# michel-aractingi/soloRL

Hardware: AMD Instinct MI355X
Metric: env-steps/s (whole node) Solo12 walk, 4096 envs/GPU (higher is better)
Workload: dtype f32

## Files before the change

### solorl_amd/csrc/dynamics.hpp

```cpp
#pragma once
#include <utility>

#include "../../include/solorl.h"
#include "../../include/solorl_model_data.h"
#include "spatial.hpp"

namespace solo {

constexpr int MAX_CONTACTS = 8;
constexpr int MAX_LIMITS = 4;
constexpr int LIM_SLOT_ROWS = 2;
constexpr int MAX_ROWS = LIM_SLOT_ROWS + 3 * MAX_CONTACTS;
SD int extra_limits(int nlt) { return nlt > LIM_SLOT_ROWS ? nlt - LIM_SLOT_ROWS : 0; }
SD int contact_cap(int nlt) { return MAX_CONTACTS - extra_limits(nlt); }
constexpr int ROW_CORE = 20;
constexpr int NPRIM = 24;
constexpr double LIMIT_WINDOW = 0.0;
constexpr double DISC_EPS2 = 1e-12;
constexpr double DISC_RIM = 0.1;

#if defined(SOLO_WAVE_TIMING) && !defined(SOLO_HOST_SHIM)
constexpr int SOLO_WT_WAVES = 65536, SOLO_WT_FIELDS = 32;
__device__ unsigned long long solo_wave_times[SOLO_WT_WAVES][SOLO_WT_FIELDS];
__shared__ unsigned long long solo_pt_acc[16];
#define SOLO_PT_DECL() long long pt_last_ = 0
#define SOLO_PT_BEGIN() do { __builtin_amdgcn_s_waitcnt(0); pt_last_ = clock64(); } while (0)
#define SOLO_PT(i) do { __builtin_amdgcn_s_waitcnt(0); if (threadIdx.x == 0) { const long long n_ = clock64(); solo_pt_acc[i] += (unsigned long long)(n_ - pt_last_); } pt_last_ = clock64(); } while (0)
#else
#define SOLO_PT_DECL() do {} while (0)
#define SOLO_PT_BEGIN() do {} while (0)
#define SOLO_PT(i) do {} while (0)
#endif

template <int N, typename F, int... I>
SD void static_for_impl(F&& f, std::integer_sequence<int, I...>) { (f(std::integral_constant<int, I>{}), ...); }
template <int N, typename F> SD void static_for(F&& f) { static_for_impl<N>(f, std::make_integer_sequence<int, N>{}); }

template <int ROBOT> struct Robot;
template <> struct Robot<0> {
  static constexpr int NJ = 2, NQ = 8, NL = 13;
  static constexpr bool SHOULDER = false;
  static constexpr const solorl_model_data& MD = SOLORL_MODEL_SOLO8;
};
template <> struct Robot<1> {
  static constexpr int NJ = 3, NQ = 12, NL = 17;
  static constexpr bool SHOULDER = true;
  static constexpr const solorl_model_data& MD = SOLORL_MODEL_SOLO12;
};

constexpr bool base_points_are_sign_patterns(const solorl_model_data& md) {
  const solorl_prim_data& a = md.prims[0]; const solorl_prim_data& b = md.prims[8];
  for (int p = 0; p < 12; p++) {
    const solorl_prim_data& q = md.prims[p];
    const bool plate = p >= 8;
    const double sx = ((plate ? (p - 8) >> 1 : p >> 2) & 1) ? -1.0 : 1.0, sy = ((plate ? (p - 8) : p >> 1) & 1) ? -1.0 : 1.0;
    const double cx = (plate ? b.center[0] : a.center[0]) * sx, cy = (plate ? b.center[1] : a.center[1]) * sy;
    const double cz = plate ? b.center[2] : ((p & 1) ? -a.center[2] : a.center[2]);
    if (q.link != 0 || q.axis != -1 || q.center[0] != cx || q.center[1] != cy || q.center[2] != cz || q.margin != a.margin || q.friction != a.friction) return false;
  }
  return true;
}

template <typename T> struct PhysParams {
  T dt, gravity, erp, slop, warm, damping, vmax, qlim, inv_dt;
  int iterations;
  T tm_hw, tm_mu;
  T resid_thr;
  T cerp;
  T cmargin;
  int mode;
  enum { M_PIPE = 1, M_URDF = 2, M_CONE = 4, M_TREADMILL = 8 };
  SD bool pgs_pipe() const { return mode & M_PIPE; }
  SD bool urdf_inertia() const { return mode & M_URDF; }
  SD bool cone() const { return mode & M_CONE; }
  SD bool tm_on() const { return mode & M_TREADMILL; }
  void set_mode(bool pipe, bool urdf, bool cone_, bool treadmill) {
    mode = (pipe ? M_PIPE : 0) | (urdf ? M_URDF : 0) | (cone_ ? M_CONE : 0) | (treadmill ? M_TREADMILL : 0);
  }
};
template <typename T> PhysParams<T> make_phys(const solorl_config& c) {
  PhysParams<T> p;
  p.dt = (T)c.sim_dt; p.gravity = (T)c.gravity; p.erp = (T)c.erp; p.slop = (T)c.linear_slop; p.warm = (T)c.warmstart;
  p.damping = (T)c.damping; p.vmax = (T)c.max_velocity; p.qlim = (T)c.joint_limit; p.inv_dt = (T)(1.0 / c.sim_dt);
  p.iterations = c.solver_iterations;
  p.tm_hw = (T)c.treadmill_half_width; p.tm_mu = (T)c.treadmill_friction;
  p.resid_thr = c.solver_residual_threshold > 0 ? (T)std::sqrt(c.solver_residual_threshold) : T(-1);
  p.cerp = (T)c.contact_erp; p.cmargin = (T)c.collision_margin;
  p.set_mode(true, c.use_urdf_inertia != 0, c.friction_model == SOLORL_FRICTION_CONE, c.use_treadmill != 0);
  return p;
}
SD int strip_feet_bits(int smask) {
  return (((smask >> 13) & 1) << 24) | (((smask >> 15) & 1) << 25) | (((smask >> 17) & 1) << 26) | (((smask >> 19) & 1) << 27);
}

template <typename T, int NQ> struct PhysState {
  V3<T> pos; T qx, qy, qz, qw; V3<T> v, w;
  T q[NQ], qd[NQ];
};

template <typename T> struct JointF { SV<T> S, U, c; T Dinv, u; };

#ifndef SOLO_HOST_SHIM
extern __shared__ __attribute__((aligned(16))) unsigned char solo_smem_sym[];
#if defined(SOLO_WAVE_TIMING)
constexpr unsigned SOLO_LDS_BASE = 128;
// ... 1812 lines not shown
    T nz = cw * z + ax * yq - ay * x + az * ww;
    T nq = cw * ww - ax * x - ay * yq - az * z;
    T inv = rsqrt_fast(nx * nx + ny * ny + nz * nz + nq * nq);
    C.ps.qx = nx * inv; C.ps.qy = ny * inv; C.ps.qz = nz * inv; C.ps.qw = nq * inv;
  }
}

template <typename T, int ROBOT, typename LDS> struct TeamCtx {
  using type = CtxLds<T, ROBOT, TeamRows<T, LDS>::off_ctx>;
  static constexpr size_t bytes = TeamRows<T, LDS>::off_ctx + 4 * sizeof(SubCtx<T, ROBOT>);
};

template <typename T, int ROBOT, typename LDS, typename CH>
SNI_SCALAR void duo_helper_rates(CH ch, const PhysParams<T> pp, const LDS lds, int t, bool valid) {
  if (valid) phase_legrates_team<T, ROBOT, LDS, CH>(ch, pp, lds, t);
  WG_SYNC();
}

template <typename T, int ROBOT>
SNI_SCALAR void duo_join_rows() {
  WG_SYNC();
}

template <typename T, int ROBOT, typename LDS, typename CH>
SNI_SCALAR void duo_integrate_joints(CH ch, const PhysParams<T> pp, const LDS lds, int t, bool valid) {
  using RB = Robot<ROBOT>;
  using TRW = TeamRows<T, LDS>;
  constexpr int NJ = RB::NJ, LN = LDS::LANES;
  if (!valid) return;
  SubCtx<T, ROBOT>& C = ch.get();
  const T dt = pp.dt;
  const int mask = C.mask;
  const int nlt = C.nlim_total;
  const T* hdr = lds.hdr();
  const SV<T> w{{hdr[2 * LN], hdr[3 * LN], hdr[4 * LN]}, {hdr[5 * LN], hdr[6 * LN], hdr[7 * LN]}};
  const int tj = t < RB::NQ ? t : 0;
  const int L = tj / NJ, k = tj - L * NJ;
  const T qds = C.qds[tj], yk = lds.y()[(L * 3 + k) * LN], qj = C.ps.q[tj];
  const SV<T> Gk = C.LR[L].G[k];
  const T* lam = TRW::lam(lds.lane);
  const int npos0 = TRW::NPOS0 + extra_limits(nlt);
  T lv[(NPRIM + 15) / 16];
#pragma unroll
  for (int i = 0; i < (NPRIM + 15) / 16; i++) {
    const int p = t + 16 * i;
    const int pp_ = p < NPRIM ? p : 0;
    lv[i] = lam[(npos0 + __builtin_popcount(mask & ((1 << pp_) - 1))) * 4];
    lv[i] = (p < NPRIM && ((mask >> pp_) & 1)) ? lv[i] : T(0);
  }
  const T nvj = clampv(qds + yk - dot(Gk, w), pp.vmax);
#pragma unroll
  for (int i = 0; i < (NPRIM + 15) / 16; i++) { const int p = t + 16 * i; if (p < NPRIM) C.lamp[p] = lv[i]; }
  if (t < RB::NQ) { C.ps.qd[t] = nvj; C.ps.q[t] = qj + dt * nvj; }
}

template <typename T, int ROBOT, typename LDS, typename CH>
SNI_SCALAR void duo_integrate_base(CH ch, const PhysParams<T> pp, const LDS lds, bool lead, bool r0) {
  constexpr int LN = LDS::LANES;
  if (!lead) return;
  SubCtx<T, ROBOT>& C = ch.get();
  const T dt = pp.dt;
  const T* hdr = lds.hdr();
  const SV<T> w{{hdr[2 * LN], hdr[3 * LN], hdr[4 * LN]}, {hdr[5 * LN], hdr[6 * LN], hdr[7 * LN]}};
  const SV<T> ub = C.ub;
  const V3<T> pos = C.ps.pos;
  const T x = C.ps.qx, yq = C.ps.qy, z = C.ps.qz, ww = C.ps.qw;
  const V3<T> nw = mk(clampv(ub.a.x + w.a.x, pp.vmax), clampv(ub.a.y + w.a.y, pp.vmax), clampv(ub.a.z + w.a.z, pp.vmax));
  const V3<T> nv = mk(clampv(ub.l.x + w.l.x, pp.vmax), clampv(ub.l.y + w.l.y, pp.vmax), clampv(ub.l.z + w.l.z, pp.vmax));
  C.ps.w = nw; C.ps.v = nv;
  C.ps.pos = fma3(nv, dt, pos);
  T wn2 = dot(nw, nw), wn = sqrt_fast(wn2), sc, s_, cw;
  sincos_t(T(0.5) * wn * dt, s_, cw);
  if (wn < T(1e-3)) sc = T(0.5) * dt - dt * dt * dt * T(1.0 / 48.0) * wn2; else sc = s_ * rcp_fast(wn);
  T ax = nw.x * sc, ay = nw.y * sc, az = nw.z * sc;
  T nx = cw * x + ax * ww + ay * z - az * yq;
  T ny = cw * yq - ax * z + ay * ww + az * x;
  T nz = cw * z + ax * yq - ay * x + az * ww;
  T nq = cw * ww - ax * x - ay * yq - az * z;
  T inv = rsqrt_fast(nx * nx + ny * ny + nz * nz + nq * nq);
  C.ps.qx = nx * inv; C.ps.qy = ny * inv; C.ps.qz = nz * inv; C.ps.qw = nq * inv;
  if (r0) C.R0 = quat_to_mat(C.ps.qx, C.ps.qy, C.ps.qz, C.ps.qw);
}

template <typename T, int ROBOT, typename LDS>
SD void substep_team_helper(const PhysParams<T> pp, const LDS& lds, int t, bool lead, bool valid, bool r0_next) {
  using CH = typename TeamCtx<T, ROBOT, LDS>::type;
  const CH ch{lds.lane};
  WG_SYNC();
  if (pp.urdf_inertia()) phase_front_team<T, ROBOT, LDS, CH, true, true>(ch, pp, lds, t, valid, lead);
  else phase_front_team<T, ROBOT, LDS, CH, false, true>(ch, pp, lds, t, valid, lead);
  WG_SYNC();
#if defined(SOLO_WAVE_TIMING)
  __builtin_amdgcn_s_waitcnt(0);
  const long long wt_h0_ = clock64();
#endif
  if (valid) team_sum_base<T, ROBOT, CH>(ch, t);
  if (lead) phase_base_lead<T, ROBOT, LDS, CH>(ch, pp, nullptr, 0u, lds);
  else if (!valid && t == 0) {
    lds.hdr()[0] = T(0); lds.hdr()[LDS::LANES] = T(0);
  }
#if defined(SOLO_WAVE_TIMING)
  __builtin_amdgcn_s_waitcnt(0);
  if (threadIdx.x == 64) solo_pt_acc[4] += (unsigned long long)(clock64() - wt_h0_);
#endif
  duo_helper_rates<T, ROBOT, LDS, CH>(ch, pp, lds, t, valid);
  duo_finish_rows<T, ROBOT, LDS, true>(pp, lds, t);
  duo_join_rows<T, ROBOT>();
  duo_join_rows<T, ROBOT>();
#if defined(SOLO_WAVE_TIMING)
  __builtin_amdgcn_s_waitcnt(0);
  const long long wt_h1_ = clock64();
#endif
  duo_integrate_base<T, ROBOT, LDS, CH>(ch, pp, lds, lead, r0_next);
#if defined(SOLO_WAVE_TIMING)
  __builtin_amdgcn_s_waitcnt(0);
  if (threadIdx.x == 64) solo_pt_acc[11] += (unsigned long long)(clock64() - wt_h1_);
#endif
}

template <typename T, int ROBOT, typename LDS, bool DUO = false>
SD int substep_team(const PhysParams<T> pp, T* lam_prev, unsigned nstride, const LDS& lds, int t, bool lead, bool valid) {
  constexpr int LN = LDS::LANES;
  using TRW = TeamRows<T, LDS>;
  using CH = typename TeamCtx<T, ROBOT, LDS>::type;
  const CH ch{lds.lane};
  SOLO_PT_DECL();
  SOLO_PT_BEGIN();
  if (valid && t < Robot<ROBOT>::NQ) {
    SubCtx<T, ROBOT>& C = ch.get();
    T sn, cs;
    sincos_t(C.ps.q[t], sn, cs);
    C.sn[t] = sn; C.cs[t] = cs;
  }
  SOLO_PT(0);
  const bool ui = pp.urdf_inertia();
  if constexpr (DUO) WG_SYNC();
  else if (ui) phase_front_team<T, ROBOT, LDS, CH, true>(ch, pp, lds, t, valid, lead);
  else phase_front_team<T, ROBOT, LDS, CH, false>(ch, pp, lds, t, valid, lead);
  SOLO_PT(1);
#if SOLO_LEG_QUAD
  if constexpr (DUO) {
    if (ui) phase_leg_rt<T, ROBOT, LDS, CH, true, true>(ch, pp, lam_prev, nstride, lds, t >> 2, t & 3);
    else phase_leg_rt<T, ROBOT, LDS, CH, false, true>(ch, pp, lam_prev, nstride, lds, t >> 2, t & 3);
  } else if (valid) {
    if (ui) phase_leg_rt<T, ROBOT, LDS, CH, true>(ch, pp, lam_prev, nstride, lds, t >> 2, t & 3);
    else phase_leg_rt<T, ROBOT, LDS, CH, false>(ch, pp, lam_prev, nstride, lds, t >> 2, t & 3);
  }
#else
  static_assert(!DUO, "the helper wavefront's barrier B is in the quad leg phase");
  if (valid && t < 4) {
    if (ui) phase_leg_rt<T, ROBOT, LDS, CH, true>(ch, pp, lam_prev, nstride, lds, t, 0);
    else phase_leg_rt<T, ROBOT, LDS, CH, false>(ch, pp, lam_prev, nstride, lds, t, 0);
  }
#endif
  SOLO_PT(2);
  if constexpr (DUO) {
    duo_join_rows<T, ROBOT>();
    SOLO_PT(3);
  } else {
    if (valid) team_sum_base<T, ROBOT, CH>(ch, t);
    SOLO_PT(3);
    if (lead) phase_base_lead<T, ROBOT, LDS, CH>(ch, pp, lam_prev, nstride, lds);
    else if (!valid && t == 0) {
      lds.hdr()[0] = T(0); lds.hdr()[LN] = T(0);
    }
    SOLO_PT(4);
    if (valid) phase_legrates_team<T, ROBOT, LDS, CH>(ch, pp, lds, t);
    SOLO_PT(5);
  }
  if constexpr (DUO) {
    duo_finish_rows<T, ROBOT, LDS, false>(pp, lds, t);
    SOLO_PT(6);
    duo_join_rows<T, ROBOT>();
    SOLO_PT(12);
  } else {
    phase_finish_team<T, ROBOT, LDS>(pp, lds, t);
    SOLO_PT(6);
  }
  phase_pgs_team<T, ROBOT, LDS>(pp.iterations, pp.warm != T(0), pp.resid_thr >= T(0), pp.pgs_pipe(), pp.cone(), lds, t);
  SOLO_PT(7);
  if constexpr (DUO) {
    duo_join_rows<T, ROBOT>();
    SOLO_PT(10);
    duo_integrate_joints<T, ROBOT, LDS, CH>(ch, pp, lds, t, valid);
  } else phase_integrate_team<T, ROBOT, LDS, CH>(ch, pp, lam_prev, nstride, lds, t, valid, lead);
  SOLO_PT(8);
  return lead ? (ch.get().mask | strip_feet_bits(ch.get().smask)) : 0;
}
#endif

// ... 26 lines not shown
```

### solorl_amd/csrc/solorl_hip.hip

```cpp
#include <hip/hip_runtime.h>

#include <cmath>
#include <cstddef>
#include <cstdio>
#include <cstdlib>
#include <cstring>
#include <utility>
#include <string>
#include <vector>

#include "../../include/solorl.h"
#include "dynamics.hpp"
#include "perturb.hpp"

using namespace solo;

#ifndef SOLO_TU_PART
#define SOLO_TU_PART -1
#endif
extern "C" __attribute__((visibility("hidden"))) int solorl_fail_(int code, const char* msg);

namespace {

#if SOLO_TU_PART == -1 || SOLO_TU_PART == 4
// ... 339 lines not shown
    E.ps = C.ps;
  }
  if (P.task == SOLORL_TASK_POINTGOAL && mode == MODE_STEP) pointgoal_progress(E, P, P.id0 + (long long)env);
  if (mode == MODE_SETTLE) { store_env(E, sf, si, L, (idx_t)N, e); return; }
  E.timestep += 1;
  const int done = reward_termination_outputs<T, NQ>(E, P, asq, out, env, N);

  if (done) reset_from_snapshot<T, ROBOT>(E, sf, L, (idx_t)N, e, env, snf, sni, M, P);
  write_obs<T, ROBOT>(E, sf, L, (idx_t)N, e, env, P.task, out.obs);
  store_env(E, sf, si, L, (idx_t)N, e);
}

#ifdef SOLO_WAVE_TIMING
#define WT_STAMP(i) do { wts_[i] = clock64(); } while (0)
#else
#define WT_STAMP(i) do {} while (0)
#endif

template <typename T> SD T team_sum16(T x) {
  if constexpr (sizeof(T) == 4) {
    x += __int_as_float(__builtin_amdgcn_mov_dpp(__float_as_int(x), 0xB1, 0xF, 0xF, true));
    x += __int_as_float(__builtin_amdgcn_mov_dpp(__float_as_int(x), 0x4E, 0xF, 0xF, true));
    x += __int_as_float(__builtin_amdgcn_mov_dpp(__float_as_int(x), 0x141, 0xF, 0xF, true));
    x += __int_as_float(__builtin_amdgcn_mov_dpp(__float_as_int(x), 0x140, 0xF, 0xF, true));
  } else {
    x += __shfl_xor(x, 1, 16); x += __shfl_xor(x, 2, 16); x += __shfl_xor(x, 4, 16); x += __shfl_xor(x, 8, 16);
  }
  return x;
}
enum { ER_GOAL = 0, ER_POT = 2, ER_PROG = 3, ER_GOALS = 4, ER_EGOALS = 5, ER_DR = 6, ER_XYPREV = 11, ER_TMY = 13, NER = 14 };
enum { IR_TIMESTEP = 0, IR_MASK = 1, IR_RNG = 2, IR_SNAP = 3, IR_DONE = 4 };
template <typename T, int ROBOT> SD void env_from_lds(Env<T, Robot<ROBOT>::NQ>& E, const SubCtx<T, ROBOT>& C) {
  E.ps = C.ps;
  E.goal[0] = C.erec[ER_GOAL]; E.goal[1] = C.erec[ER_GOAL + 1]; E.pot = C.erec[ER_POT]; E.prog = C.erec[ER_PROG];
  E.goals = C.erec[ER_GOALS]; E.egoals = C.erec[ER_EGOALS];
#pragma unroll
  for (int k = 0; k < 5; k++) E.dr[k] = C.erec[ER_DR + k];
  E.xyprev[0] = C.erec[ER_XYPREV]; E.xyprev[1] = C.erec[ER_XYPREV + 1]; E.tmy = C.erec[ER_TMY];
  E.timestep = C.irec[IR_TIMESTEP]; E.mask = C.irec[IR_MASK]; E.rng = C.irec[IR_RNG];
}
template <typename T, int ROBOT> SD void scalars_to_lds(const Env<T, Robot<ROBOT>::NQ>& E, SubCtx<T, ROBOT>& C) {
  C.erec[ER_GOAL] = E.goal[0]; C.erec[ER_GOAL + 1] = E.goal[1]; C.erec[ER_POT] = E.pot; C.erec[ER_PROG] = E.prog;
  C.erec[ER_GOALS] = E.goals; C.erec[ER_EGOALS] = E.egoals;
#pragma unroll
  for (int k = 0; k < 5; k++) C.erec[ER_DR + k] = E.dr[k];
  C.erec[ER_XYPREV] = E.xyprev[0]; C.erec[ER_XYPREV + 1] = E.xyprev[1]; C.erec[ER_TMY] = E.tmy;
  C.irec[IR_TIMESTEP] = E.timestep; C.irec[IR_MASK] = E.mask; C.irec[IR_RNG] = E.rng;
}

template <typename T, int ROBOT, int HK_>
SD void team_current_state(const SubCtx<T, ROBOT>& C, int task, int D, int t, T (&cs)[HK_]) {
  constexpr int NQ = Robot<ROBOT>::NQ;
  using PS_ = PhysState<T, NQ>;
  static_assert(offsetof(PS_, v) == 7 * sizeof(T) && offsetof(PS_, q) == 13 * sizeof(T) && sizeof(PS_) == (13 + 2 * NQ) * sizeof(T),
                "PhysState is a flat array: pos 0-2, quat 3-6, v 7-9, w 10-12, q, qd");
  const T* psv = reinterpret_cast<const T*>(&C.ps);
  const int mask = C.irec[IR_MASK];
  const T g0 = C.erec[ER_GOAL], g1 = C.erec[ER_GOAL + 1];
  T ang = T(0);
  if (t >= 1 && t <= 3) {
    T r, p, y;
    euler_zyx(C.ps.qx, C.ps.qy, C.ps.qz, C.ps.qw, r, p, y);
    const T a = t == 1 ? r : (t == 2 ? p : y);
    ang = (a - T(2) * floor(a * T(0.5))) * T(0.5);
  }
#pragma unroll
  for (int k = 0; k < HK_; k++) {
    const int d = t + 16 * k;
    const int e = d - (14 + 2 * NQ);
    const int idx = d == 0 ? 2 : (d < 10 + 2 * NQ ? d + 3 : (e >= 0 && e < 2 ? e : 0));
    const T raw = psv[idx];
    const T sc = d < 10 ? T(1) : (d < 10 + NQ ? T(0.1) : (d < 10 + 2 * NQ ? T(0.01) : T(0.5)));
    T v = raw * sc;
    if (d >= 1 && d <= 3) v = ang;
    const int f = d - (10 + 2 * NQ);
    if (f >= 0 && f < 4) v = ((mask >> (13 + 2 * f)) & 1) ? T(1) : T(0);
    if (e == 2) v = g0 * T(0.5);
    if (e == 3) v = g1 * T(0.5);
    if (task != SOLORL_TASK_POINTGOAL && e >= 0) v = T(0);
    cs[k] = d < D ? v : T(0);
  }
}

constexpr float POL_HALF_LOG_2PI = 0.91893853320467274178f;
constexpr unsigned POL_ENV_BYTES = 2496;
static_assert(POL_ENV_BYTES == MAX_ROWS * (ROW_CORE + 4) * sizeof(float), "the policy tail's per-env slice is one env's fp32 row storage (RowLds)");
static_assert((224 + 128) * sizeof(float) <= POL_ENV_BYTES, "the last activation block (h2: 128 floats at float offset 224) must end inside the slice");
SD float pol_tanh(float x) { const float e = __expf(2.0f * x); return 1.0f - 2.0f * __builtin_amdgcn_rcpf(1.0f + e); }
typedef float nfloat4 __attribute__((ext_vector_type(4)));
typedef __attribute__((address_space(1))) const nfloat4 gfloat4;
SD float pol_dot4(nfloat4 w, nfloat4 x, float acc) { return fmaf(w.x, x.x, fmaf(w.y, x.y, fmaf(w.z, x.z, fmaf(w.w, x.w, acc)))); }
#define POL_PIN4(x) asm volatile("" : "+v"(x))
template <int KB> struct PolBatch { nfloat4 c[KB], a[KB]; };
template <int KB>
SD void pol_load(PolBatch<KB>& B, const float* wc_, const float* wa_, int K4, int k0, int lane) {
  gfloat4* wc = (gfloat4*)(wc_ + (size_t)lane * 4 * K4);
  gfloat4* wa = (gfloat4*)(wa_ + (size_t)lane * 4 * K4);
#pragma unroll
  for (int kk = 0; kk < KB; kk++) {
    const int k = k0 + kk < K4 ? k0 + kk : K4 - 1;
    B.c[kk] = wc[k]; B.a[kk] = wa[k];
  }
  asm volatile("" ::: "memory");
}
template <int KB>
SD void pol_fma(PolBatch<KB>& B, int K4, int k0, unsigned xoff, unsigned xoff_a, float (&c)[4], float (&a)[4]) {
  asm volatile("" ::: "memory");
#pragma unroll
  for (int kk = 0; kk < KB; kk++) { POL_PIN4(B.c[kk]); POL_PIN4(B.a[kk]); }
#pragma unroll
  for (int kk = 0; kk < KB; kk++)
    if (k0 + kk < K4) {
#pragma unroll
      for (int e = 0; e < 4; e++) {
        const nfloat4 xc = reinterpret_cast<const nfloat4*>(solo_smem + e * POL_ENV_BYTES + xoff)[k0 + kk];
        const nfloat4 xa = xoff_a == xoff ? xc : reinterpret_cast<const nfloat4*>(solo_smem + e * POL_ENV_BYTES + xoff_a)[k0 + kk];
        c[e] = pol_dot4(B.c[kk], xc, c[e]); a[e] = pol_dot4(B.a[kk], xa, a[e]);
      }
    }
}
SD void pol_act_store(const float (&c)[4], const float (&a)[4], unsigned yoff, int lane) {
#pragma unroll
  for (int e = 0; e < 4; e++) {
    float* y = reinterpret_cast<float*>(solo_smem + e * POL_ENV_BYTES + yoff);
    y[lane] = pol_tanh(c[e]); y[64 + lane] = pol_tanh(a[e]);
  }
}

template <int A>
SD void policy_tail_team(const PolicyTail& P, int O, int col, int t, idx_t env, bool valid) {
  float* const buf = reinterpret_cast<float*>(solo_smem + (unsigned)col * POL_ENV_BYTES);
  float* const h2 = buf + 224;
  const int lane = threadIdx.x & 63, O4 = O >> 2;
  static_assert(A < 15, "the critic head sits on lane 15");
  const bool head = t < A || t == 15;
  constexpr unsigned H1 = 96u * 4u, H2 = 224u * 4u;
  float c[4], a[4];
  PolBatch<11> w1a, w1b;
  PolBatch<8> w2a, w2b;
  nfloat4 whb[16];
  pol_load(w1a, P.cw0, P.aw0, O4, 0, lane);
  pol_load(w1b, P.cw0, P.aw0, O4, 11, lane);
#pragma unroll
  for (int e = 0; e < 4; e++) { c[e] = P.cb0[lane]; a[e] = P.ab0[lane]; }
  pol_fma(w1a, O4, 0, 0u, 0u, c, a);
  pol_load(w2a, P.cw1, P.aw1, 16, 0, lane);
  pol_fma(w1b, O4, 11, 0u, 0u, c, a);
  pol_act_store(c, a, H1, lane);
  pol_load(w2b, P.cw1, P.aw1, 16, 8, lane);
#pragma unroll
  for (int e = 0; e < 4; e++) { c[e] = P.cb1[lane]; a[e] = P.ab1[lane]; }
  TEAM_SYNC();
  pol_fma(w2a, 16, 0, H1, H1 + 256u, c, a);
  {
    gfloat4* wh = (gfloat4*)(t == 15 ? P.cw2 : P.mw + (size_t)(head ? t : 0) * 64);
#pragma unroll
    for (int k = 0; k < 16; k++) whb[k] = wh[k];
    asm volatile("" ::: "memory");
  }
  pol_fma(w2b, 16, 8, H1, H1 + 256u, c, a);
  pol_act_store(c, a, H2, lane);
  TEAM_SYNC();
  float out = 0.f;
  {
    asm volatile("" ::: "memory");
#pragma unroll
    for (int k = 0; k < 16; k++) POL_PIN4(whb[k]);
    const nfloat4* x = reinterpret_cast<const nfloat4*>(t == 15 ? h2 : h2 + 64);
    float o0 = t == 15 ? P.cb2[0] : P.mb[head ? t : 0], o1 = 0.f;
#pragma unroll
    for (int k = 0; k < 16; k += 2) { o0 = pol_dot4(whb[k], x[k], o0); o1 = pol_dot4(whb[k + 1], x[k + 1], o1); }
    out = head ? o0 + o1 : 0.f;
  }
  float lp = 0.f, act = out;
  if (t < A) {
    const float ls = P.logstd[t];
    const float nz = P.noise ? P.noise[(size_t)env * A + t] : 0.f;
    act = out + __expf(ls) * nz;
    lp = -0.5f * nz * nz - ls - POL_HALF_LOG_2PI;
  }
  lp = team_sum16(lp);
  if (valid) {
    if (t < A) P.action[(size_t)env * A + t] = act;
    if (t == 15) P.value[env] = out;
    if (t == 0) P.logp[env] = lp;
  }
}

template <typename T, int ROBOT, bool DUO = false>
SD void step_team(T* __restrict__ sf, int* __restrict__ si, const T* __restrict__ snf, const int* __restrict__ sni, int M,
                  const Layout& L, int N, const EnvParams& P, const PhysParams<T>& pp, const float* __restrict__ actions,
                  const Outputs& out, int mode) {
  using RB = Robot<ROBOT>;
  constexpr int NQ = RB::NQ, NPS = 13 + 2 * NQ;
  using LDS = RowLds<T, 4>;
  using CH = typename TeamCtx<T, ROBOT, LDS>::type;
  static_assert(sizeof(PhysState<T, NQ>) == NPS * sizeof(T), "PhysState is the HBM field order pos, quat, v, w, q, qd");
#ifdef SOLO_WAVE_TIMING
  long long wts_[11];
  for (int i_ = 0; i_ < 11; i_++) wts_[i_] = 0;
  const long long wr0_ = wall_clock64();
  if (threadIdx.x < 16) solo::solo_pt_acc[threadIdx.x] = 0;
  __syncthreads();
  wts_[0] = clock64();
#endif
  const unsigned wlane = DUO ? (threadIdx.x & 63u) : threadIdx.x;
  const int t = wlane & 15, col = wlane >> 4;
  const unsigned blk = (blockIdx.x & 7u) * (gridDim.x >> 3) + (blockIdx.x >> 3);
  idx_t e = (idx_t)blk * 4 + col;
  const bool valid = e < (idx_t)N;
  if (!valid) e = (idx_t)N - 1;
  const bool lead = valid && t == 0;
  LDS lds; lds.lanes = 4; lds.lane = col;
  if (P.lds_poison_on) {
    using TC = TeamCtx<T, ROBOT, LDS>;
    unsigned* w = reinterpret_cast<unsigned*>(solo_smem);
    for (unsigned k = wlane; k < TC::bytes / 4; k += 64) w[k] = P.lds_poison;
    __syncthreads();
  }
  const CH ch{col};
  SubCtx<T, ROBOT>& C = ch.get();
  T* const psv = reinterpret_cast<T*>(&C.ps);
  if constexpr (DUO) {
    if (blk * 4u >= (unsigned)N) return;
    if (__builtin_amdgcn_readfirstlane(threadIdx.x >> 6)) {
#pragma unroll 1
      for (int ss = 0; ss < P.frame_skip; ss++)
        substep_team_helper<T, ROBOT>(pp, lds, t, lead, valid, ss + 1 < P.frame_skip);
      duo_join_rows<T, ROBOT>();
      return;
    }
    if (!valid && t == 0) { C.mask = 0; C.nc = 0; C.nlim_total = 0; C.lsel = 0; C.smask = 0; }
  }
  idx_t env = 0;
  T a_t = T(0);
  if (valid) {
    env = P.linear_ids ? e : (idx_t)si[SX(I_ENVID, e, NI)];
    for (int f = t; f < NPS; f += 16) psv[f] = sf[SX(L.pos + f, e, L.NF)];
    if (t < NER) C.erec[t] = sf[SX(L.goal + t, e, L.NF)];
    if (t < 3) C.irec[t] = si[SX(t, e, NI)];
    for (int p = t; p < NPRIM; p += 16) C.lamp[p] = sf[SX(L.lam + p, e, L.NF)];
    if (t < NQ && mode == MODE_STEP) a_t = (T)actions[env * NQ + t];
  }
  static_assert(I_TIMESTEP == IR_TIMESTEP && I_MASK == IR_MASK && I_RNG == IR_RNG, "counter order");
  TEAM_SYNC();
  WT_STAMP(1);
  if (valid && t < NQ) {
    const T c = a_t < T(-1) ? T(-1) : (a_t > T(1) ? T(1) : a_t);
    T tq;
    if (P.control == SOLORL_CONTROL_TORQUE) tq = c * T(P.max_torque);
    else tq = clampv(T(P.kp) * (c * pp.qlim - C.ps.q[t]) - T(P.kd) * C.ps.qd[t], T(P.max_torque));
    C.tau_base[t] = mode == MODE_STEP ? tq : T(0);
    if (out.tau && mode == MODE_STEP) out.tau[env * NQ + t] = (float)tq;
  }
  const T asq = team_sum16(a_t * a_t);
  WT_STAMP(2);
  constexpr int HK = (DMAX + 15) / 16;
  T hk0[HK], hk1[HK];
#pragma unroll
  for (int k = 0; k < HK; k++) { hk0[k] = T(0); hk1[k] = T(0); }
  T csk[HK];
  if (L.H > 0) team_current_state<T, ROBOT, HK>(C, P.task, L.D, t, csk);
  TEAM_SYNC();
  if (lead) {
    C.erec[ER_XYPREV] = C.ps.pos.x; C.erec[ER_XYPREV + 1] = C.ps.pos.y;
    C.tmy = C.erec[ER_TMY];
    if constexpr (DUO) C.R0 = quat_to_mat(C.ps.qx, C.ps.qy, C.ps.qz, C.ps.qw);
  }
  if (valid && L.H > 0) {
#pragma unroll
    for (int k = 0; k < HK; k++) {
      const int d = t + 16 * k;
      if (d < L.D) {
        const T c = csk[k];
        for (int lv = L.H - 1; lv >= 2; lv--)
          sf[SX(L.hist + lv * HSTRIDE + d, e, L.NF)] = sf[SX(L.hist + (lv - 1) * HSTRIDE + d, e, L.NF)];
        if (L.H >= 2) { hk1[k] = sf[SX(L.hist + d, e, L.NF)]; sf[SX(L.hist + HSTRIDE + d, e, L.NF)] = hk1[k]; }
        sf[SX(L.hist + d, e, L.NF)] = c;
        hk0[k] = c;
      } else if (d < ((L.D + 3) & ~3)) {
        sf[SX(L.hist + d, e, L.NF)] = T(0);
        for (int lv = 1; lv < L.H; lv++) sf[SX(L.hist + lv * HSTRIDE + d, e, L.NF)] = T(0);
      }
    }
  }
  WT_STAMP(3);
#pragma unroll 1
  for (int ss = 0; ss < P.frame_skip; ss++) {
    const T sc = (ss == 0 || P.hold_torque) ? T(1) : T(0);
    if (valid && t < NQ) C.tau[t] = C.tau_base[t] * sc;
    const int m = substep_team<T, ROBOT, LDS, DUO>(pp, sf + SX(L.lam, e, L.NF), 4u, lds, t, lead, valid);
    if (lead) C.irec[IR_MASK] = m;
  }
  if constexpr (DUO) {
    duo_join_rows<T, ROBOT>();
  }
  WT_STAMP(4);
  if (valid) for (int p = t; p < NPRIM; p += 16) sf[SX(L.lam + p, e, L.NF)] = C.lamp[p];
  WT_STAMP(5);
  if (lead) {
    Env<T, NQ> E;
    env_from_lds<T, ROBOT>(E, C);
    int done = 0;
    if (P.task == SOLORL_TASK_POINTGOAL && mode == MODE_STEP) pointgoal_progress(E, P, P.id0 + (long long)env);
    if (mode == MODE_STEP) {
      E.timestep += 1;
      done = reward_termination_outputs<T, NQ>(E, P, asq, out, env, N);
      if (done) C.irec[IR_SNAP] = reset_draws(E, P, P.id0 + (long long)env);
    }
    scalars_to_lds<T, ROBOT>(E, C);
    C.irec[IR_DONE] = done;
  }
  WT_STAMP(6);
  TEAM_SYNC();
  const int done = valid ? C.irec[IR_DONE] : 0;
  if (done) {
    const idx_t k = (idx_t)C.irec[IR_SNAP], MM = (idx_t)M;
    for (int f = t; f < L.NF; f += 16) {
      const T v = snf[SX(f, k, L.NF)];
      const bool scalar = f >= L.goal && f < L.goal + NER;
      if (!scalar) sf[SX(f, e, L.NF)] = v;
      if (f < NPS) psv[f] = v;
      else if (scalar && f != L.goal && f != L.goal + 1) C.erec[f - L.goal] = v;
    }
    if (t == 1) C.irec[IR_MASK] = sni[SX(I_MASK, k, NI)];
#pragma unroll
    for (int kk = 0; kk < HK; kk++) {
      const int d = t + 16 * kk;
      if (d < L.D) {
        if (L.H >= 1) hk0[kk] = snf[SX(L.hist + d, k, L.NF)];
        if (L.H >= 2) hk1[kk] = snf[SX(L.hist + HSTRIDE + d, k, L.NF)];
      }
    }
    TEAM_SYNC();
    const T g0 = C.erec[ER_GOAL], g1 = C.erec[ER_GOAL + 1];
    if (P.task == SOLORL_TASK_POINTGOAL) {
#pragma unroll
      for (int kk = 0; kk < HK; kk++) {
        const int d = t + 16 * kk;
        if (d == L.D - 2 || d == L.D - 1) {
          const T gv = (d == L.D - 2 ? g0 : g1) * T(0.5);
          if (L.H >= 1) { hk0[kk] = gv; sf[SX(L.hist + d, e, L.NF)] = gv; }
          if (L.H >= 2) { hk1[kk] = gv; sf[SX(L.hist + HSTRIDE + d, e, L.NF)] = gv; }
          for (int lv = 2; lv < L.H; lv++) sf[SX(L.hist + lv * HSTRIDE + d, e, L.NF)] = gv;
        }
      }
    }
    if (t == 0) {
      C.irec[IR_TIMESTEP] = 0;
      C.erec[ER_GOALS] = T(0); C.erec[ER_EGOALS] = T(0);
#pragma unroll
      for (int q = 0; q < 5; q++) C.erec[ER_DR + q] = T(0);
      if (P.task == SOLORL_TASK_POINTGOAL) {
        const T dx = C.ps.pos.x - g0, dy = C.ps.pos.y - g1, px = C.erec[ER_XYPREV] - g0, py = C.erec[ER_XYPREV + 1] - g1;
        const T pot = sqrt(dx * dx + dy * dy);
        C.erec[ER_POT] = pot; C.erec[ER_PROG] = -(pot - sqrt(px * px + py * py));
      }
    }
  }
  WT_STAMP(7);
  const bool want_obs = mode == MODE_STEP;
  TEAM_SYNC();
  T cso[HK];
  if (want_obs) team_current_state<T, ROBOT, HK>(C, P.task, L.D, t, cso);
  WT_STAMP(8);
  bool with_policy = false;
  if constexpr (sizeof(T) == 4) with_policy = want_obs && out.pol.value != nullptr;
  if (valid) {
    if (want_obs) {
      float* o = out.obs + env * (idx_t)(L.D * (1 + L.H));
      float* ol = reinterpret_cast<float*>(solo_smem + (unsigned)col * POL_ENV_BYTES);
#pragma unroll
      for (int k = 0; k < HK; k++) {
        const int d = t + 16 * k;
        if (d < L.D) {
          const T c = cso[k];
          o[d] = (float)c;
          if (L.H >= 1) o[L.D + d] = (float)(c - hk0[k]);
          if (L.H >= 2) o[2 * L.D + d] = (float)(c - hk1[k]);
          for (int lv = 2; lv < L.H; lv++) {
            T hv;
            if (done) {
              hv = snf[SX(L.hist + lv * HSTRIDE + d, (idx_t)C.irec[IR_SNAP], L.NF)];
              if (P.task == SOLORL_TASK_POINTGOAL && d >= L.D - 2) hv = C.erec[ER_GOAL + (d - (L.D - 2))] * T(0.5);
            } else hv = sf[SX(L.hist + lv * HSTRIDE + d, e, L.NF)];
            o[(lv + 1) * L.D + d] = (float)(c - hv);
          }
          if (with_policy) {
            ol[d] = (float)c;
            if (L.H >= 1) ol[L.D + d] = (float)(c - hk0[k]);
          }
        }
      }
    }
    for (int f = t; f < ((NPS + 3) & ~3); f += 16) sf[SX(L.pos + f, e, L.NF)] = f < NPS ? psv[f] : T(0);
    sf[SX(L.goal + t, e, L.NF)] = t < NER ? C.erec[t] : T(0);
    if (t < 3) si[SX(t, e, NI)] = C.irec[t];
  }
  if constexpr (sizeof(T) == 4) {
    if (with_policy) {
      TEAM_SYNC();
      policy_tail_team<NQ>(out.pol, L.D * (1 + L.H), col, t, env, valid);
    }
  }
  WT_STAMP(9);
#ifdef SOLO_WAVE_TIMING
  __builtin_amdgcn_s_waitcnt(0);
  if (threadIdx.x == 0 && blockIdx.x < solo::SOLO_WT_WAVES) {
    wts_[10] = clock64();
    unsigned long long* w_ = solo::solo_wave_times[blockIdx.x];
    w_[0] = (unsigned long long)(wts_[3] - wts_[0]); w_[1] = (unsigned long long)(wts_[4] - wts_[3]); w_[2] = (unsigned long long)(wts_[10] - wts_[4]);
    w_[3] = (unsigned long long)(wall_clock64() - wr0_);
    for (int i_ = 0; i_ < 10; i_++) w_[6 + i_] = (unsigned long long)(wts_[i_ + 1] > wts_[i_] && wts_[i_] ? wts_[i_ + 1] - wts_[i_] : 0);
    for (int i_ = 0; i_ < 10; i_++) w_[16 + i_] = solo::solo_pt_acc[i_];
    for (int i_ = 10; i_ < 14; i_++) w_[18 + i_] = solo::solo_pt_acc[i_];
  }
#endif
}

template <typename T, int ROBOT>
__global__ void __launch_bounds__(64)
step_kernel(T* __restrict__ sf, int* __restrict__ si, const T* __restrict__ snf, const int* __restrict__ sni, int M,
            Layout L, int N, EnvParams P, PhysParams<T> pp, const float* __restrict__ actions, Outputs out, int mode) {
  step_body<T, ROBOT>(sf, si, snf, sni, M, L, N, P, pp, actions, out, mode);
}

#ifndef SOLO_WAVES_PER_SIMD
#define SOLO_WAVES_PER_SIMD 2
#endif
template <typename T, int ROBOT>
__global__ void __launch_bounds__(64, sizeof(T) == 8 ? 1 : SOLO_WAVES_PER_SIMD)
step_kernel_team(T* __restrict__ sf, int* __restrict__ si, const T* __restrict__ snf, const int* __restrict__ sni, int M,
                 Layout L, int N, EnvParams P, PhysParams<T> pp, const float* __restrict__ actions, Outputs out, int mode) {
  step_team<T, ROBOT>(sf, si, snf, sni, M, L, N, P, pp, actions, out, mode);
}

template <typename T, int ROBOT>
__global__ void __launch_bounds__(128, SOLO_WAVES_PER_SIMD)
duo_kernel_team(T* __restrict__ sf, int* __restrict__ si, const T* __restrict__ snf, const int* __restrict__ sni, int M,
                Layout L, int N, EnvParams P, PhysParams<T> pp, const float* __restrict__ actions, Outputs out, int mode) {
  static_assert(sizeof(T) == 4, "the helper wavefront is an fp32 kernel");
  step_team<T, ROBOT, true>(sf, si, snf, sni, M, L, N, P, pp, actions, out, mode);
}

template <typename T> struct RolloutArgs {
  T* sf; int* si; const T* snf; const int* sni; int M;
  Layout L; int N; EnvParams P; PhysParams<T> pp;
  const float* actions; Outputs out;
  int mode;
  int K, pol_last;
};
template <typename T> SD T* row_adv(T* p, size_t n) { return p ? p + n : p; }
template <typename T, int ROBOT>
__global__ void __launch_bounds__(64, sizeof(T) == 8 ? 1 : SOLO_WAVES_PER_SIMD)
rollout_kernel_team(const RolloutArgs<T> args) {
  using RA = RolloutArgs<T>;
  typedef const __attribute__((address_space(4))) char* kptr;
  constexpr size_t A = Robot<ROBOT>::NQ;
  const int K = args.K;
#pragma unroll 1
  for (int k = 0; k < K; k++) {
    kptr ap = (kptr)__builtin_amdgcn_kernarg_segment_ptr();
    asm volatile("" : "+s"(ap));
    const RA& a = *(const RA*)ap;
    const size_t r = (size_t)k * (size_t)a.N, O = (size_t)(a.L.D * (1 + a.L.H));
    Outputs o = a.out;
    o.obs += r * O; o.rew += r; o.done += r;
    o.timeout = row_adv(o.timeout, r); o.success = row_adv(o.success, r); o.nan_reset = row_adv(o.nan_reset, r);
    o.ep_len = row_adv(o.ep_len, r); o.ep_rew = row_adv(o.ep_rew, r); o.goals = row_adv(o.goals, r);
    o.dr0 = row_adv(o.dr0, r); o.dr1 = row_adv(o.dr1, r); o.dr2 = row_adv(o.dr2, r); o.dr3 = row_adv(o.dr3, r); o.dr4 = row_adv(o.dr4, r);
    o.tau = row_adv(o.tau, r * A);
    if (o.pol.value) {
      if (k + 1 < K || a.pol_last) {
        const size_t r1 = r + (size_t)a.N;
        o.pol.value += r1; o.pol.logp += r1; o.pol.action += r1 * A; o.pol.noise = row_adv(o.pol.noise, r1 * A);
      } else o.pol.value = nullptr;
    }
    step_team<T, ROBOT>(a.sf, a.si, a.snf, a.sni, a.M, a.L, a.N, a.P, a.pp, a.actions + r * A, o, a.mode);
    TEAM_SYNC();
  }
}

template <typename T, int ROBOT, bool MASKED>
__global__ void reset_kernel(T* sf, int* si, const T* snf, const int* sni, int M, Layout L, int N, EnvParams P, float* obs,
                             const unsigned char* mask) {
  const idx_t e = (idx_t)blockIdx.x * blockDim.x + threadIdx.x;
  if (e >= (idx_t)N) return;
  if constexpr (MASKED) { if (!mask[si[SX(I_ENVID, e, NI)]]) return; }
  Env<T, Robot<ROBOT>::NQ> E;
  load_env(E, sf, si, L, (idx_t)N, e);
  const idx_t env = (idx_t)si[SX(I_ENVID, e, NI)];
  reset_from_snapshot<T, ROBOT>(E, sf, L, (idx_t)N, e, env, snf, sni, M, P);
  if (obs) write_obs<T, ROBOT>(E, sf, L, (idx_t)N, e, env, P.task, obs);
  store_env(E, sf, si, L, (idx_t)N, e);
  si[SX(I_NEEDRESET, e, NI)] = 0;
}

template <typename T, int ROBOT>
// ... 312 lines not shown
  Layout L;
  void* sf = nullptr; int* si = nullptr; void* snf = nullptr; int* sni = nullptr;
  void* sf2 = nullptr; int* si2 = nullptr; int* perm = nullptr;
  bool sort = true;
  uint64_t seed = 0; int64_t id0 = 0;
  double goal_radius = 2.0;
  double* dyn = nullptr;
  std::vector<unsigned> stab_host;
  unsigned* stab = nullptr;
  bool spread = true;
  bool team = false;
  int lds_poison_on = 0; unsigned lds_poison = 0;
  int simds = 1024;
  int pipe_override = -1;
  int helper_override = -1;
  int* pert_countdown = nullptr; unsigned* pert_kicks = nullptr;
  PerturbParams pert{};
};

namespace {

EnvParams make_env_params(const solorl_env* h) {
  EnvParams P;
  const solorl_config& c = h->cfg;
  P.task = c.task; P.control = c.control; P.frame_skip = c.frame_skip; P.episode_length = c.episode_length;
  P.hold_torque = c.hold_torque; P.disable_termination = c.disable_termination;
  P.settle_min = c.settle_min; P.nsettle = c.settle_max - c.settle_min + 1;
  P.seed_lo = (unsigned)h->seed; P.seed_hi = (unsigned)(h->seed >> 32); P.id0 = h->id0;
  P.kp = c.kp; P.kd = c.kd; P.max_torque = c.max_torque; P.reward_dt = c.reward_dt; P.dyn = h->dyn;
  P.lds_poison_on = h->lds_poison_on; P.lds_poison = h->lds_poison;
  P.use_treadmill = c.use_treadmill; P.tm_offset = (float)c.treadmill_offset;
  P.linear_ids = h->sort ? 0 : 1;
  return P;
}

inline int check_lds_base(const void* kernel) {
  hipFuncAttributes a;
  HIP_TRY(hipFuncGetAttributes(&a, kernel));
  if (a.sharedSizeBytes != (size_t)SOLO_LDS_BASE)
    return fail(SOLORL_ERR_HIP, "step kernel's static LDS size differs from SOLO_LDS_BASE: the phase functions' dynamic-LDS base constant does not hold "
                                "(a -DSOLO_WAVE_TIMING build runs team mode only)");
  return 0;
}

inline int team_grid(int N) { return (((N + 3) / 4) + 7) & ~7; }
inline bool team_pipe(const solorl_env* h, int N) { return h->pipe_override >= 0 ? h->pipe_override != 0 : team_grid(N) <= h->simds; }
inline bool helper_wave_allowed(const solorl_env* h) { return h->team && !h->f64 && !h->sort && team_grid(h->N) <= h->simds; }
inline bool helper_wave_rule(const solorl_env* h) { return h->helper_override != 0 && helper_wave_allowed(h); }
inline bool step_n_one_launch(const solorl_env* h) { return h->team && !h->sort; }

template <typename T, int ROBOT>
PhysParams<T> team_launch_shape(const solorl_env* h, int N, dim3& grid, size_t& smem) {
  grid = dim3(team_grid(N));
  using TeamLds = RowLds<T, 4>;
  smem = TeamCtx<T, ROBOT, TeamLds>::bytes;
  static_assert(sizeof(T) == 8 || TeamCtx<T, ROBOT, TeamLds>::bytes <= 20480, "team-mode LDS must allow 8 workgroups per CU (two wavefronts per SIMD)");
  PhysParams<T> pp = make_phys<T>(h->cfg);
  pp.mode = (pp.mode & ~PhysParams<T>::M_PIPE) | (team_pipe(h, N) ? PhysParams<T>::M_PIPE : 0);
  return pp;
}

template <typename T, int ROBOT>
int prepare_kernels(const solorl_env* h) {
  if (int rc = check_lds_base(h->team ? reinterpret_cast<const void*>(step_kernel_team<T, ROBOT>) : reinterpret_cast<const void*>(step_kernel<T, ROBOT>))) return rc;
  if constexpr (sizeof(T) == 4)
    if (helper_wave_rule(h))
      if (int rc = check_lds_base(reinterpret_cast<const void*>(duo_kernel_team<T, ROBOT>))) return rc;
  if (step_n_one_launch(h))
    if (int rc = check_lds_base(reinterpret_cast<const void*>(rollout_kernel_team<T, ROBOT>))) return rc;
  if (!h->team)
    HIP_TRY(hipFuncSetAttribute(reinterpret_cast<const void*>(step_kernel<T, ROBOT>), hipFuncAttributeMaxDynamicSharedMemorySize,
                                (int)RowLds<T>::bytes(sizeof(T) == 8 ? 32 : 64)));
  return 0;
}

template <typename T, int ROBOT>
int launch_step(solorl_env* h, T* sf, int* si, int N, const float* actions, const Outputs& out, int mode, hipStream_t st) {
  if (h->team) {
    dim3 grid;
    size_t team_smem = 0;
    const PhysParams<T> pp = team_launch_shape<T, ROBOT>(h, N, grid, team_smem);
    if constexpr (sizeof(T) == 4) {
      if (helper_wave_rule(h)) {
        hipLaunchKernelGGL((duo_kernel_team<T, ROBOT>), grid, dim3(128), team_smem, st, sf, si, (const T*)h->snf, (const int*)h->sni, h->M, h->L, N,
                           make_env_params(h), pp, actions, out, mode);
        HIP_TRY(hipGetLastError());
        return 0;
      }
    }
    hipLaunchKernelGGL((step_kernel_team<T, ROBOT>), grid, dim3(64), team_smem, st, sf, si, (const T*)h->snf, (const int*)h->sni, h->M, h->L, N,
                       make_env_params(h), pp, actions, out, mode);
    HIP_TRY(hipGetLastError());
    return 0;
  }
  const int EPB = RowLds<T>::LANES;
  size_t smem = RowLds<T>::bytes(EPB);
  if (h->spread && (N + EPB - 1) / EPB <= 256) smem = RowLds<T>::bytes(sizeof(T) == 8 ? 32 : 64);
  dim3 grid((N + EPB - 1) / EPB), block(EPB);
  hipLaunchKernelGGL((step_kernel<T, ROBOT>), grid, block, smem, st, sf, si, (const T*)h->snf, (const int*)h->sni, h->M, h->L, N,
                     make_env_params(h), make_phys<T>(h->cfg), actions, out, mode);
  HIP_TRY(hipGetLastError());
  return 0;
}

template <typename T, int ROBOT>
int launch_rollout(solorl_env* h, T* sf, int* si, int N, const float* actions, const Outputs& out, int K, int pol_last, hipStream_t st) {
  dim3 grid, block(64);
  RolloutArgs<T> a;
  size_t smem = 0;
  a.pp = team_launch_shape<T, ROBOT>(h, N, grid, smem);
  a.sf = sf; a.si = si; a.snf = (const T*)h->snf; a.sni = (const int*)h->sni; a.M = h->M; a.L = h->L; a.N = N; a.P = make_env_params(h);
  a.actions = actions; a.out = out; a.mode = MODE_STEP; a.K = K; a.pol_last = pol_last;
  hipLaunchKernelGGL((rollout_kernel_team<T, ROBOT>), grid, block, smem, st, a);
  HIP_TRY(hipGetLastError());
  return 0;
}

}

#define SOLO_LAUNCH_ARGS solorl_env* h, void* sf, int* si, int N, const float* actions, const void* out, int mode, void* st
#define SOLO_ROLLOUT_ARGS solorl_env* h, void* sf, int* si, int N, const float* actions, const void* out, int K, int pol_last, void* st
#define SOLO_DECLARE_PART(K_) \
  extern "C" __attribute__((visibility("hidden"))) int solorl_prepare_part##K_(const solorl_env* h); \
  extern "C" __attribute__((visibility("hidden"))) int solorl_launch_part##K_(SOLO_LAUNCH_ARGS); \
  extern "C" __attribute__((visibility("hidden"))) int solorl_rollout_part##K_(SOLO_ROLLOUT_ARGS);
SOLO_DECLARE_PART(0) SOLO_DECLARE_PART(1) SOLO_DECLARE_PART(2) SOLO_DECLARE_PART(3)
#define SOLO_DEFINE_PART(K_, T_, R_) \
  extern "C" int solorl_prepare_part##K_(const solorl_env* h) { return prepare_kernels<T_, R_>(h); } \
  extern "C" int solorl_launch_part##K_(SOLO_LAUNCH_ARGS) { \
    return launch_step<T_, R_>(h, (T_*)sf, si, N, actions, *(const Outputs*)out, mode, (hipStream_t)st); } \
  extern "C" int solorl_rollout_part##K_(SOLO_ROLLOUT_ARGS) { \
    return launch_rollout<T_, R_>(h, (T_*)sf, si, N, actions, *(const Outputs*)out, K, pol_last, (hipStream_t)st); }
#if SOLO_TU_PART == -1 || SOLO_TU_PART == 0
SOLO_DEFINE_PART(0, float, 0)
#endif
#if SOLO_TU_PART == -1 || SOLO_TU_PART == 1
SOLO_DEFINE_PART(1, float, 1)
#endif
#if SOLO_TU_PART == -1 || SOLO_TU_PART == 2
SOLO_DEFINE_PART(2, double, 0)
#endif
#if SOLO_TU_PART == -1 || SOLO_TU_PART == 3
SOLO_DEFINE_PART(3, double, 1)
#endif

#if SOLO_TU_PART == -1 || SOLO_TU_PART == 4
namespace {

template <typename F> auto with_type(const solorl_env* h, F&& f) { return h->f64 ? f(double{}) : f(float{}); }
template <typename F> auto with_instantiation(const solorl_env* h, F&& f) {
  return with_type(h, [&](auto t) {
    return h->cfg.robot == SOLORL_ROBOT_SOLO12 ? f(t, std::integral_constant<int, 1>{}) : f(t, std::integral_constant<int, 0>{});
  });
}

int part_index(const solorl_env* h) { return 2 * (h->f64 ? 1 : 0) + (h->cfg.robot == SOLORL_ROBOT_SOLO12 ? 1 : 0); }
constexpr decltype(&solorl_launch_part0) PART_LAUNCH[4] = {solorl_launch_part0, solorl_launch_part1, solorl_launch_part2, solorl_launch_part3};
constexpr decltype(&solorl_rollout_part0) PART_ROLLOUT[4] = {solorl_rollout_part0, solorl_rollout_part1, solorl_rollout_part2, solorl_rollout_part3};
constexpr decltype(&solorl_prepare_part0) PART_PREPARE[4] = {solorl_prepare_part0, solorl_prepare_part1, solorl_prepare_part2, solorl_prepare_part3};

int dispatch_step(solorl_env* h, void* sf, int* si, int N, const float* actions, const Outputs& out, int mode, hipStream_t st) {
  return PART_LAUNCH[part_index(h)](h, sf, si, N, actions, &out, mode, st);
}

int dispatch_rollout(solorl_env* h, const float* actions, const Outputs& out, int K, int pol_last, hipStream_t st) {
  return PART_ROLLOUT[part_index(h)](h, h->sf, h->si, h->N, actions, &out, K, pol_last, st);
}
// ... 588 lines not shown
```

Measured before the change: 29.19 million.

## Offload observation-history state build to helper wave and prefetch step inputs in duo kernel

In the two-wave duo kernel, the helper wave now computes the current-state observation vector during its first substep, between the two row joins, and writes it to a new LDS area. The main wave then reads it after the join instead of computing it inline and synchronising. The main wave also batch-loads pose, goal, integer, lambda and history values into registers up front, pinned with asm barriers, so those memory loads are issued together. In exchange the duo launch uses more dynamic LDS, guarded by a static_assert meant to keep 8 workgroups per CU, and the history-shift code is duplicated.

Result: no change. 29.41 million (median of 6 runs) (+0.7%).

```diff
diff --git a/solorl_amd/csrc/dynamics.hpp b/solorl_amd/csrc/dynamics.hpp
--- a/solorl_amd/csrc/dynamics.hpp
+++ b/solorl_amd/csrc/dynamics.hpp
@@ -20,7 +20,7 @@
 constexpr double DISC_RIM = 0.1;
 
 #if defined(SOLO_WAVE_TIMING) && !defined(SOLO_HOST_SHIM)
-constexpr int SOLO_WT_WAVES = 65536, SOLO_WT_FIELDS = 32;
+constexpr int SOLO_WT_WAVES = 65536, SOLO_WT_FIELDS = 36;
 __device__ unsigned long long solo_wave_times[SOLO_WT_WAVES][SOLO_WT_FIELDS];
 __shared__ unsigned long long solo_pt_acc[16];
 #define SOLO_PT_DECL() long long pt_last_ = 0
@@ -1999,8 +1999,8 @@
   if (r0) C.R0 = quat_to_mat(C.ps.qx, C.ps.qy, C.ps.qz, C.ps.qw);
 }
 
-template <typename T, int ROBOT, typename LDS>
-SD void substep_team_helper(const PhysParams<T> pp, const LDS& lds, int t, bool lead, bool valid, bool r0_next) {
+template <typename T, int ROBOT, typename LDS, typename PRE>
+SD void substep_team_helper(const PhysParams<T> pp, const LDS& lds, int t, bool lead, bool valid, bool r0_next, const PRE pre) {
   using CH = typename TeamCtx<T, ROBOT, LDS>::type;
   const CH ch{lds.lane};
   WG_SYNC();
@@ -2023,6 +2023,14 @@
   duo_helper_rates<T, ROBOT, LDS, CH>(ch, pp, lds, t, valid);
   duo_finish_rows<T, ROBOT, LDS, true>(pp, lds, t);
   duo_join_rows<T, ROBOT>();
+#if defined(SOLO_WAVE_TIMING)
+  const long long wt_h2_ = clock64();
+#endif
+  pre();
+#if defined(SOLO_WAVE_TIMING)
+  __builtin_amdgcn_s_waitcnt(0);
+  if (threadIdx.x == 64) solo_pt_acc[14] += (unsigned long long)(clock64() - wt_h2_);
+#endif
   duo_join_rows<T, ROBOT>();
 #if defined(SOLO_WAVE_TIMING)
   __builtin_amdgcn_s_waitcnt(0);
diff --git a/solorl_amd/csrc/solorl_hip.hip b/solorl_amd/csrc/solorl_hip.hip
--- a/solorl_amd/csrc/solorl_hip.hip
+++ b/solorl_amd/csrc/solorl_hip.hip
@@ -445,6 +445,26 @@
   }
 }
 
+template <typename T, int ROBOT> struct DuoPre {
+  static constexpr int HK = (DMAX + 15) / 16;
+  static constexpr size_t off = TeamCtx<T, ROBOT, RowLds<T, 4>>::bytes;
+  static constexpr size_t bytes = off + 4 * 16 * HK * sizeof(T);
+  SD static T* area(int col) { return reinterpret_cast<T*>(solo_smem + off) + col * 16 * HK; }
+};
+template <typename T, int ROBOT>
+SNI_SCALAR void duo_pre_state(int task, int D, bool valid) {
+  constexpr int HK = DuoPre<T, ROBOT>::HK;
+  const int t = threadIdx.x & 15, col = (threadIdx.x & 63u) >> 4;
+  if (!valid) return;
+  const typename TeamCtx<T, ROBOT, RowLds<T, 4>>::type ch{col};
+  T cs[HK];
+  team_current_state<T, ROBOT, HK>(ch.get(), task, D, t, cs);
+  T* const a = DuoPre<T, ROBOT>::area(col);
+#pragma unroll
+  for (int k = 0; k < HK; k++) a[t + 16 * k] = cs[k];
+}
+#define DUO_PIN(x) asm volatile("" : "+v"(x))
+
 constexpr float POL_HALF_LOG_2PI = 0.91893853320467274178f;
 constexpr unsigned POL_ENV_BYTES = 2496;
 static_assert(POL_ENV_BYTES == MAX_ROWS * (ROW_CORE + 4) * sizeof(float), "the policy tail's per-env slice is one env's fp32 row storage (RowLds)");
@@ -560,8 +580,8 @@
   using CH = typename TeamCtx<T, ROBOT, LDS>::type;
   static_assert(sizeof(PhysState<T, NQ>) == NPS * sizeof(T), "PhysState is the HBM field order pos, quat, v, w, q, qd");
 #ifdef SOLO_WAVE_TIMING
-  long long wts_[11];
-  for (int i_ = 0; i_ < 11; i_++) wts_[i_] = 0;
+  long long wts_[12];
+  for (int i_ = 0; i_ < 12; i_++) wts_[i_] = 0;
   const long long wr0_ = wall_clock64();
   if (threadIdx.x < 16) solo::solo_pt_acc[threadIdx.x] = 0;
   __syncthreads();
@@ -579,6 +599,8 @@
     using TC = TeamCtx<T, ROBOT, LDS>;
     unsigned* w = reinterpret_cast<unsigned*>(solo_smem);
     for (unsigned k = wlane; k < TC::bytes / 4; k += 64) w[k] = P.lds_poison;
+    if constexpr (DUO)
+      for (unsigned k = TC::bytes / 4 + wlane; k < DuoPre<T, ROBOT>::bytes / 4; k += 64) w[k] = P.lds_poison;
     __syncthreads();
   }
   const CH ch{col};
@@ -587,9 +609,13 @@
   if constexpr (DUO) {
     if (blk * 4u >= (unsigned)N) return;
     if (__builtin_amdgcn_readfirstlane(threadIdx.x >> 6)) {
+      const int pre_task = L.H > 0 ? P.task : -1, pre_D = L.D;
 #pragma unroll 1
       for (int ss = 0; ss < P.frame_skip; ss++)
-        substep_team_helper<T, ROBOT>(pp, lds, t, lead, valid, ss + 1 < P.frame_skip);
+        substep_team_helper<T, ROBOT>(pp, lds, t, lead, valid, ss + 1 < P.frame_skip,
+                                      [ss, pre_task, pre_D, valid]() __attribute__((always_inline)) {
+          if (ss == 0 && pre_task >= 0) duo_pre_state<T, ROBOT>(pre_task, pre_D, valid);
+        });
       duo_join_rows<T, ROBOT>();
       return;
     }
@@ -597,7 +623,41 @@
   }
   idx_t env = 0;
   T a_t = T(0);
-  if (valid) {
+  constexpr int HK = (DMAX + 15) / 16;
+  T hold[HK];
+  if constexpr (DUO) {
+    constexpr int KPS = (NPS + 15) / 16, KLP = (NPRIM + 15) / 16;
+    T ps_[KPS], lp_[KLP], er_ = T(0);
+    int ir_ = 0;
+#pragma unroll
+    for (int k = 0; k < HK; k++) hold[k] = T(0);
+    if (valid) {
+      env = P.linear_ids ? e : (idx_t)si[SX(I_ENVID, e, NI)];
+#pragma unroll
+      for (int k = 0; k < KPS; k++) ps_[k] = sf[SX(L.pos + (t + 16 * k < NPS ? t + 16 * k : t), e, L.NF)];
+      er_ = sf[SX(L.goal + (t < NER ? t : 0), e, L.NF)];
+      ir_ = si[SX(t < 3 ? t : 0, e, NI)];
+#pragma unroll
+      for (int k = 0; k < KLP; k++) lp_[k] = sf[SX(L.lam + (t + 16 * k < NPRIM ? t + 16 * k : t), e, L.NF)];
+      if (L.H >= 2) {
+#pragma unroll
+        for (int k = 0; k < HK; k++) hold[k] = sf[SX(L.hist + (t + 16 * k < L.D ? t + 16 * k : t), e, L.NF)];
+      }
+      if (t < NQ && mode == MODE_STEP) a_t = (T)actions[env * NQ + t];
+      asm volatile("" ::: "memory");
+#pragma unroll
+      for (int k = 0; k < KPS; k++) DUO_PIN(ps_[k]);
+      DUO_PIN(er_); DUO_PIN(ir_);
+#pragma unroll
+      for (int k = 0; k < KLP; k++) DUO_PIN(lp_[k]);
+#pragma unroll
+      for (int k = 0; k < KPS; k++) if (t + 16 * k < NPS) psv[t + 16 * k] = ps_[k];
+      if (t < NER) C.erec[t] = er_;
+      if (t < 3) C.irec[t] = ir_;
+#pragma unroll
+      for (int k = 0; k < KLP; k++) if (t + 16 * k < NPRIM) C.lamp[t + 16 * k] = lp_[k];
+    }
+  } else if (valid) {
     env = P.linear_ids ? e : (idx_t)si[SX(I_ENVID, e, NI)];
     for (int f = t; f < NPS; f += 16) psv[f] = sf[SX(L.pos + f, e, L.NF)];
     if (t < NER) C.erec[t] = sf[SX(L.goal + t, e, L.NF)];
@@ -618,19 +678,20 @@
   }
   const T asq = team_sum16(a_t * a_t);
   WT_STAMP(2);
-  constexpr int HK = (DMAX + 15) / 16;
   T hk0[HK], hk1[HK];
 #pragma unroll
   for (int k = 0; k < HK; k++) { hk0[k] = T(0); hk1[k] = T(0); }
   T csk[HK];
-  if (L.H > 0) team_current_state<T, ROBOT, HK>(C, P.task, L.D, t, csk);
-  TEAM_SYNC();
+  if constexpr (!DUO) {
+    if (L.H > 0) team_current_state<T, ROBOT, HK>(C, P.task, L.D, t, csk);
+    TEAM_SYNC();
+  }
   if (lead) {
     C.erec[ER_XYPREV] = C.ps.pos.x; C.erec[ER_XYPREV + 1] = C.ps.pos.y;
     C.tmy = C.erec[ER_TMY];
     if constexpr (DUO) C.R0 = quat_to_mat(C.ps.qx, C.ps.qy, C.ps.qz, C.ps.qw);
   }
-  if (valid && L.H > 0) {
+  if (!DUO && valid && L.H > 0) {
 #pragma unroll
     for (int k = 0; k < HK; k++) {
       const int d = t + 16 * k;
@@ -657,6 +718,25 @@
   }
   if constexpr (DUO) {
     duo_join_rows<T, ROBOT>();
+    WT_STAMP(11);
+    if (valid && L.H > 0) {
+      const T* const pre = DuoPre<T, ROBOT>::area(col);
+#pragma unroll
+      for (int k = 0; k < HK; k++) {
+        const int d = t + 16 * k;
+        if (d < L.D) {
+          const T c = pre[d];
+          for (int lv = L.H - 1; lv >= 2; lv--)
+            sf[SX(L.hist + lv * HSTRIDE + d, e, L.NF)] = sf[SX(L.hist + (lv - 1) * HSTRIDE + d, e, L.NF)];
+          if (L.H >= 2) { hk1[k] = hold[k]; sf[SX(L.hist + HSTRIDE + d, e, L.NF)] = hk1[k]; }
+          sf[SX(L.hist + d, e, L.NF)] = c;
+          hk0[k] = c;
+        } else if (d < ((L.D + 3) & ~3)) {
+          sf[SX(L.hist + d, e, L.NF)] = T(0);
+          for (int lv = 1; lv < L.H; lv++) sf[SX(L.hist + lv * HSTRIDE + d, e, L.NF)] = T(0);
+        }
+      }
+    }
   }
   WT_STAMP(4);
   if (valid) for (int p = t; p < NPRIM; p += 16) sf[SX(L.lam + p, e, L.NF)] = C.lamp[p];
@@ -777,6 +857,8 @@
     for (int i_ = 0; i_ < 10; i_++) w_[6 + i_] = (unsigned long long)(wts_[i_ + 1] > wts_[i_] && wts_[i_] ? wts_[i_ + 1] - wts_[i_] : 0);
     for (int i_ = 0; i_ < 10; i_++) w_[16 + i_] = solo::solo_pt_acc[i_];
     for (int i_ = 10; i_ < 14; i_++) w_[18 + i_] = solo::solo_pt_acc[i_];
+    w_[32] = solo::solo_pt_acc[14];
+    w_[33] = (unsigned long long)(wts_[11] ? wts_[4] - wts_[11] : 0);
   }
 #endif
 }
@@ -1255,7 +1337,9 @@
     const PhysParams<T> pp = team_launch_shape<T, ROBOT>(h, N, grid, team_smem);
     if constexpr (sizeof(T) == 4) {
       if (helper_wave_rule(h)) {
-        hipLaunchKernelGGL((duo_kernel_team<T, ROBOT>), grid, dim3(128), team_smem, st, sf, si, (const T*)h->snf, (const int*)h->sni, h->M, h->L, N,
+        static_assert(DuoPre<T, ROBOT>::bytes <= 20480, "the duo kernel's LDS must allow 8 workgroups per CU, as team mode's");
+        const size_t duo_smem = DuoPre<T, ROBOT>::bytes;
+        hipLaunchKernelGGL((duo_kernel_team<T, ROBOT>), grid, dim3(128), duo_smem, st, sf, si, (const T*)h->snf, (const int*)h->sni, h->M, h->L, N,
                            make_env_params(h), pp, actions, out, mode);
         HIP_TRY(hipGetLastError());
         return 0;
```
